# gphocs-dev/G-PhoCS

Measured on AMD Instinct MI355X. Metric: locus-likelihood evals/sec (+ MCMC iters/sec), 100k loci, 1/2/4/8 MI355X, higher is better.
Workload: dtype f64

## Files before the change

g-phocs_amd/__init__.py:

```python
import ctypes as C
import os
import subprocess

import numpy as np

from .synth import make_synthetic_pack, replicate_pack, write_pack

_HERE = os.path.dirname(os.path.abspath(__file__))
REPO = os.path.dirname(_HERE)
LIB_PATH = os.path.join(_HERE, "libgphocs_hip.so")
CSRC = os.path.join(_HERE, "csrc")

HIPCC_BASE = ["--offload-arch=gfx950", "-O3", "-std=c++17", "-ffp-contract=off", "-fPIC", "-shared",
              "-Wno-unused-result", "-pthread"]
HIPCC_TUNING = ["-mllvm", "-disable-machine-licm", "-mllvm", "-structurizecfg-skip-uniform-regions",
                "-mllvm", "-amdgpu-sched-strategy=max-ilp"]
HIPCC_TUNING_SPILLING = HIPCC_TUNING[:4]
HIPCC_FLAGS = HIPCC_BASE + HIPCC_TUNING
HIPCC_LIBS = ["-ldl", "-lrt"]
HIPCC_VALIDATED = "roc-7.2.0 26014"
PLAIN_LIB = "libgphocs_hip_plain.so"
CHECKED_LIB = "libgphocs_hip_chk.so"
CHECKED_LIB_BIG = "libgphocs_hip_chkb.so"

# ... 195 lines not shown
    "gph_control_sample_name", "gph_loci_read", "gph_loci_free", "gph_loci_arrays", "gph_run_control_file", "gph_run_control_file_ranked",
    "gph_read_trace", "gph_engine_locus_rate_update", "gph_engine_set_locus_rates", "gph_mcmc_set_locus_rate_finetune",
    "gph_mcmc_locus_rate_state", "gph_engine_set_comm", "gph_engine_host_stats", "gph_engine_set_timing",
    "gph_comm_unique_id", "gph_comm_create_rccl", "gph_comm_create_shm", "gph_comm_attach_shm", "gph_comm_shm_bytes",
    "gph_comm_destroy", "gph_comm_world", "gph_comm_rank", "gph_comm_on_stream", "gph_comm_kind",
    "gph_comm_allgather_stream", "gph_comm_allreduce_host", "gph_run_control_file_comm", "gph_device_count",
    "gph_engine_unit", "gph_build_id", "gph_build_compiler", "gph_runtime_version", "gph_engine_steplog_enable", "gph_engine_steplog_fetch", "gph_comm_local_group", "gph_comm_create_local",
    "gph_mcmc_get_chain", "gph_mcmc_set_chain", "gph_mcmc_update_gb", "gph_mcmc_update_locus_rate", "gph_mcmc_update_theta",
    "gph_mcmc_update_mig_rates", "gph_mcmc_update_tau", "gph_mcmc_update_sample_age", "gph_mcmc_mixing",
    "gph_mcmc_synchronize_events", "gph_mcmc_check_all", "gph_mcmc_initialize_genealogies",
    "gph_engine_locus_summary_enable", "gph_engine_locus_summary_sample", "gph_engine_locus_summary_columns",
    "gph_engine_locus_summary_fetch", "gph_engine_locus_summary_column_name", "gph_loci_name", "gph_run_control_file_ex",
    "gph_engine_coal_stats_enable", "gph_engine_coal_stats_sample", "gph_engine_coal_stats_shape", "gph_engine_coal_stats_fetch",
    "gph_engine_coal_stats_column_name", "gph_run_control_file_ex2", "gph_coal_stats_write", "gph_coal_stats_discard",
    "gph_engine_coal_stats_set_chunk", "gph_coal_stats_combined",
]


_LIBS = {}


def load_library(path=None, dims=None):
    if path is None and dims is not None:
        path = lib_path(variant_for(*dims))
    path = path or LIB_PATH
    if path in _LIBS:
        return _LIBS[path]
    lib = _load_library(path)
    _LIBS[path] = lib
    return lib
# ... 84 lines not shown
    lib.gph_engine_locus_summary_column_name.argtypes = [C.c_void_p, C.c_int32]
    lib.gph_engine_locus_summary_column_name.restype = C.c_char_p
    lib.gph_loci_name.argtypes = [C.c_void_p, C.c_int64]
    lib.gph_loci_name.restype = C.c_char_p
    lib.gph_run_control_file_ex.argtypes = [C.c_char_p, C.c_char_p, C.c_int32, C.c_int32, C.c_void_p, C.c_char_p]
    lib.gph_engine_coal_stats_enable.argtypes = [C.c_void_p, C.c_int32]
    lib.gph_engine_coal_stats_sample.argtypes = [C.c_void_p, C.c_int32]
    lib.gph_engine_coal_stats_shape.argtypes = [C.c_void_p] + [C.POINTER(C.c_int32)] * 4
    lib.gph_engine_coal_stats_fetch.argtypes = [C.c_void_p, C.POINTER(C.c_double), C.c_int32, C.POINTER(C.c_int32)]
    lib.gph_engine_coal_stats_column_name.argtypes = [C.c_void_p, C.c_int32]
    lib.gph_engine_coal_stats_column_name.restype = C.c_char_p
    lib.gph_run_control_file_ex2.argtypes = [C.c_char_p, C.c_char_p, C.c_int32, C.c_int32, C.c_void_p, C.c_char_p, C.c_char_p, C.c_int32]
    lib.gph_coal_stats_write.argtypes = [C.c_char_p, C.c_int32]
    lib.gph_coal_stats_discard.argtypes = [C.c_char_p, C.c_int32]
    lib.gph_engine_coal_stats_set_chunk.argtypes = [C.c_void_p, C.c_int32]
    lib.gph_coal_stats_combined.argtypes = [C.c_char_p, C.c_int32, C.POINTER(C.c_double), C.c_int64, C.POINTER(C.c_int64), C.POINTER(C.c_int32)]
    return lib


def encode_phases(counts):
    a = np.asarray(counts, dtype=np.int64)
    big = a >= 0x8000
    if big.any():
        ex = np.round(np.log2(np.where(big, a, 1))).astype(np.int64)
        assert np.all((1 << ex[big]) == a[big]), "a phase count of 2^15 or more must be a power of two"
        a = np.where(big, 0x8000 | ex, a)
    return a.astype(np.uint16)


def decode_phases(words):
# ... 332 lines not shown
    def last_kernel_ms(self, which):
        ms = C.c_double()
        self._chk(self.lib.gph_engine_last_kernel_ms(self.engine, which, C.byref(ms)), "kernel_ms")
        return ms.value

    def class_stats(self, which, reset=False):
        o = (C.c_double * 5)()
        self._chk(self.lib.gph_engine_class_stats(self.engine, which, o, int(reset)), "class_stats")
        return dict(launches=o[0], ms=o[1], evals=o[2], bytes=o[3], nodes=o[4])

    def host_stats(self):
        a, b, c, r = C.c_int64(), C.c_int64(), C.c_int64(), C.c_int32()
        self._chk(self.lib.gph_engine_host_stats(self.engine, C.byref(a), C.byref(b), C.byref(c), C.byref(r)), "host_stats")
        return dict(syncs=a.value, collectives=b.value, launches=c.value, resident=bool(r.value))

    def set_timing(self, mask):
        self._chk(self.lib.gph_engine_set_timing(self.engine, mask), "set_timing")

    def unit(self, op, arg=0):
        stride = max(13, 3 * (self.pack.n - 1), 1 + 5 * (2 * self.pack.n - 1))
        out = np.zeros((self.end - self.begin, stride))
        self._chk(self.lib.gph_engine_unit(self.engine, op, arg, out.ctypes.data_as(C.POINTER(C.c_double)), stride), "unit")
        return out

    def debug_oob(self):
        w, c = C.c_int32(), C.c_int32()
        self._chk(self.lib.gph_engine_debug_oob(self.engine, C.byref(w), C.byref(c)), "debug_oob")
        return w.value, c.value

    def enable_locus_summary(self, on=True):
# ... 66 lines not shown
```

g-phocs_amd/csrc/gph_engine.hip:

```cpp
#include <stdio.h>
#include <stdlib.h>
#include <stddef.h>
#include <string.h>
#include <vector>
#include <string>
#include <algorithm>
#if defined(GPH_HOSTEMU) && defined(GPH_EMU64)
#define GPH_EMU64_IMPL
#endif
#include "gph_kernels.h"
#include "gph_global.h"
#include "gph_summary.h"
#include "gph_coalstats.h"
#include "gph_comm.h"
#include "../../include/gphocs_hip.h"

#ifdef GPH_HOSTEMU
thread_local char *gph_sm = nullptr;
thread_local GphLds gph_lds;
GphLayout g_lay;
GphModel g_model;
GphGlobal *gph_G_emu = nullptr;
#ifdef GPH_BOUNDS
int gph_oob_word = 0;
// ... 326 lines not shown
  bool sync_pending = false;
  bool fin_owed = false;
  bool mix_owed = false;
  int32_t slog_sel = 0;
  bool mirror_current = true;
  bool no_fuse = false;
  gph_counters counters = {0, 0, 0.0, 0};
  double *d_ls = nullptr;
  int32_t ls_ncol = 0;
  int64_t ls_samples = 0;
  std::vector<std::string> ls_names;
  double *d_cs_part = nullptr, *d_cs_rows = nullptr;
  int32_t cs_cap = 0, cs_fill = 0, cs_rd = 0, cs_chunk = 0, cs_nchunks = 0, cs_bd = 0;
  int32_t cs_chunk_next = 0;
  std::string cs_name;
  double last_ms[16] = {0};
  double cls_launches[16] = {0}, cls_ms[16] = {0};
  double cls_evals0[16] = {0}, cls_bytes0[16] = {0}, cls_nodes0[16] = {0};
  int last_which = 0;
  uint32_t timing_mask = 0xffffffffu;
#ifndef GPH_HOSTEMU
  hipStream_t stream = nullptr;
  hipStream_t stream_wide = nullptr;
  hipEvent_t ev_fork = nullptr, ev_join = nullptr;
  bool side_stream = true;
  struct Tm { hipEvent_t a, b; int which; };
  std::vector<Tm> tm;
  size_t tm_used = 0;
#else
  std::vector<char> lds;
// ... 517 lines not shown
  e->popFather.assign(cfg->popFather, cfg->popFather + cfg->K);
  e->popSon0.assign(cfg->popSon0, cfg->popSon0 + cfg->K);
  e->popSon1.assign(cfg->popSon1, cfg->popSon1 + cfg->K);
  if (cfg->B > 0) { e->bandSrc.assign(cfg->bandSrc, cfg->bandSrc + cfg->B); e->bandTgt.assign(cfg->bandTgt, cfg->bandTgt + cfg->B); }
  e->cfg.samplesPerPop = e->samplesPerPop.data();
  e->cfg.popFather = e->popFather.data();
  e->cfg.popSon0 = e->popSon0.data();
  e->cfg.popSon1 = e->popSon1.data();
  e->cfg.bandSrc = e->bandSrc.data();
  e->cfg.bandTgt = e->bandTgt.data();
  memset(&e->dev, 0, sizeof e->dev);
  memset(&e->ka, 0, sizeof e->ka);
  fill_math_constants(e->ka);
  if (const char *fh = getenv("GPH_HOST_DECISIONS")) e->force_host = atoi(fh) != 0;
  if (const char *nf = getenv("GPH_NO_FUSE")) e->no_fuse = atoi(nf) != 0;
#ifndef GPH_HOSTEMU
  int ndev = 0;
  if (hipGetDeviceCount(&ndev) != hipSuccess || ndev <= cfg->device) {
    fprintf(stderr, "gphocs_hip: no usable HIP device %d (found %d) -- this library has no CPU path\n", cfg->device, ndev);
    delete e;
    return GPH_EHIP;
  }
  if (hipSetDevice(cfg->device) != hipSuccess || fill_math_tables(e->ka)) {
    fprintf(stderr, "gphocs_hip: cannot resolve the device math tables\n");
    delete e;
    return GPH_EHIP;
  }
  if (const char *ov = getenv("GPH_SIDE_STREAM")) e->side_stream = atoi(ov) != 0;
  const bool nb_ = getenv("GPH_NONBLOCKING_STREAM") && atoi(getenv("GPH_NONBLOCKING_STREAM")) != 0;
  if ((nb_ ? hipStreamCreateWithFlags(&e->stream, hipStreamNonBlocking) : hipStreamCreate(&e->stream)) != hipSuccess ||
// ... 15 lines not shown
  e->d_gather = e->d_red;
#endif
  memset(e->G_h, 0, sizeof(GphGlobal));
  e->G_h->error_locus = -1;
  build_model_static(e);
  *out = e;
  return 0;
}

void gph_engine_destroy(gph_engine *e)
{
  if (!e) return;
  dev_free(e->dev.pages); dev_free(e->dev.shadow); dev_free(e->dev.cond); dev_free((void *)e->dev.cond_off);
  dev_free((void *)e->dev.seq); dev_free((void *)e->dev.seq_off); dev_free((void *)e->dev.orig); dev_free((void *)e->dev.P); dev_free(e->dev.out); dev_free(e->dev.stats); dev_free(e->d_mutRate);
  dev_free(e->d_lrec); dev_free(e->d_lpre); dev_free(e->d_slot_of); dev_free(e->d_lr_result); dev_free(e->d_lr_gscr); dev_free(e->d_ref_page); dev_free(e->d_ref_seq);
  dev_free(e->d_part); dev_free(e->dev.err); dev_free(e->d_ls); dev_free(e->d_cs_part); dev_free(e->d_cs_rows);
  for (void *p : e->deferred_free) dev_free(p);
  e->deferred_free.clear();
  dev_free((void *)e->dev.slog_map); dev_free(e->dev.slog); dev_free(e->dev.slog_n);
  if (e->d_gather != e->d_red) dev_free(e->d_gather);
  dev_free(e->d_red);
#ifdef GPH_HOSTEMU
  free(e->h_red);
  free(e->G_h);
#else
  dev_free(e->G_d);
  dev_free(e->d_ticket);
  if (e->h_red) (void)hipHostFree(e->h_red);
  if (e->G_h) (void)hipHostFree(e->G_h);
  for (auto &t : e->tm) { (void)hipEventDestroy(t.a); (void)hipEventDestroy(t.b); }
  if (e->ev_fork) (void)hipEventDestroy(e->ev_fork);
// ... 270 lines not shown
  e->cs_fill = 0;
  LAUNCH(e, 3, k_init, e->seedz, (const double *)e->d_mutRate, e->init_predraws);
  int rc = reduce_local(e, 0, GPH_OUT_SLOTS);
  if (!rc) rc = reduce_stats(e);
  if (rc) return rc;
  e->G_h->nrec = 0;
  e->G_h->iteration = -1;
  if ((rc = run_stage_now(e, GS_INIT_DONE, 0))) return rc;
  { GphRed R; R.rows = e->h_red; R.world = 1;
    if (sumGen) *sumGen = R.sum(0, 0);
    if (sumData) *sumData = R.sum(0, 1); }
  e->initialized = true;
  return rc;
}

int gph_engine_genealogy_sweep(gph_engine *e, int32_t flags, double ftCoal, double ftMig, gph_sweep_result *out)
{
  if (!e || !e->initialized || !out) return GPH_ESTATE;
  SETDEV(e);
  PUSH_IF_DIRTY(e);
  const int with_sync = e->sync_pending ? 8 : 0;
  e->sync_pending = false;
  GphGlobal &G = *e->G_h;
  const double d0 = G.dataLogLikelihood, l0 = G.logLikelihood;
  const int64_t a0 = G.acc[0], a1 = G.acc[1], a2 = G.acc[2], a7 = G.acc[7];
  int with_mix = 0;
  if (e->mix_owed) {
    if (!e->mirror_current) { int rcm = finish_sync(e); if (rcm) return rcm; }
    e->mix_owed = false;
    if (e->G_h->mix_flag) with_mix = 16;
  }
  LAUNCH(e, 0, k_sweep, (int)flags | with_sync | with_mix, ftCoal, ftMig, e->G_h->mix_c, e->G_h->mix_lnc);
  int rc = reduce_local(e, 0, GPH_OUT_SLOTS);
  if (!rc) rc = reduce_stats(e);
  if (rc) return rc;
  if ((rc = run_stage_now(e, GS_SWEEP_DONE, with_sync))) return rc;
  GphRed R; R.rows = e->h_red; R.world = 1;
  out->accepted_internal = G.acc[0] - a0;
  out->accepted_mignode = G.acc[1] - a1;
  out->accepted_spr = G.acc[2] - a2;
  out->total_mig_nodes = G.acc[7] - a7;
  out->dData_internal = R.sum(0, 3);
  out->dLog_internal = R.sum(0, 4);
  out->dLog_mignode = R.sum(0, 5);
  out->dData_spr = R.sum(0, 6);
  out->dLog_spr = R.sum(0, 7);
// ... 232 lines not shown

int gph_engine_host_stats(gph_engine *e, int64_t *syncs, int64_t *collectives, int64_t *launches, int32_t *resident_mode)
{
  if (!e) return GPH_EARG;
  if (syncs) *syncs = e->n_syncs;
  if (collectives) *collectives = e->n_collectives;
  if (launches) *launches = e->n_launches;
  if (resident_mode) *resident_mode = resident(e) ? 1 : 0;
  return 0;
}
int gph_engine_set_timing(gph_engine *e, uint32_t class_mask)
{
  if (!e) return GPH_EARG;
  e->timing_mask = class_mask;
  return 0;
}

int gph_debug_math(const double *x, const double *y, int32_t n, double *out, int32_t device)
{
  if (!x || !y || !out || n <= 0) return GPH_EARG;
#ifdef GPH_HOSTEMU
  (void)device;
  for (int i = 0; i < n; i++) {
    out[i] = gph_exp(x[i]); out[n + i] = gph_log(x[i]); out[2 * n + i] = sqrt(fabs(x[i]));
    out[3 * n + i] = x[i] / y[i]; out[4 * n + i] = floor(x[i]);
  }
  return 0;
#else
  double *dx = nullptr, *dy = nullptr, *dout = nullptr;
  HIPCHK(hipSetDevice(device));
// ... 86 lines not shown
  *nrec = n;
#ifdef GPH_BBCOUNT
  n = e->dev.slog_cap;
#endif
  const int32_t m = std::min(std::min(n, e->dev.slog_cap), max_records);
  if (out && m > 0 && d2h(e, out, e->dev.slog + (size_t)idx * e->dev.slog_cap * 8, sizeof(double) * 8 * (size_t)m)) return GPH_EHIP;
  if (reset) { const int32_t z = 0; if (h2d(e, e->dev.slog_n + idx, &z, sizeof z)) return GPH_EHIP; }
  return 0;
#endif
}

int gph_engine_hbm_bytes(gph_engine *e, double *bytes)
{
  if (!e || !bytes) return GPH_EARG;
  *bytes = 2.0 * e->pages_bytes + (double)e->cond_bytes + (double)e->seq_bytes_total + 8.0 * GPH_OUT_SLOTS * e->L;
  return 0;
}

int gph_engine_set_locus_rates(gph_engine *e, const double *rates, int32_t draws, int32_t variable)
{
  if (!e || !e->loaded || e->initialized || !rates || draws < 0) return GPH_ESTATE;
  SETDEV(e);
  std::vector<double> r(e->L);
  for (int64_t j = 0; j < e->L; j++) r[j] = rates[e->h_orig[j]];
  if (!e->d_mutRate && dev_alloc((void **)&e->d_mutRate, sizeof(double) * e->L)) return GPH_EHIP;
  if (h2d(e, e->d_mutRate, r.data(), sizeof(double) * e->L)) return GPH_EHIP;
  e->init_predraws = draws;
  e->var_rates = variable != 0;
  return 0;
}
// ... 185 lines not shown
{
  if (e->fin_owed) { e->fin_owed = false; LAUNCH(e, 5, k_tau_finish, 0); }
  return 0;
}
static int part_sweep(gph_engine *e, int32_t iteration, double ftCoal, double ftMig)
{
  int rc;
  const int with_sync = e->sync_pending ? 8 : 0;
  e->sync_pending = false;
  int with_mix = 0;
  if (e->mix_owed) {
    if (!e->mirror_current) { int rcm = finish_sync(e); if (rcm) return rcm; }
    e->mix_owed = false;
    if (e->G_h->mix_flag) with_mix = 16;
  }
  LAUNCH(e, 0, k_sweep, 7 | with_sync | with_mix, ftCoal, ftMig, e->G_h->mix_c, e->G_h->mix_lnc);
  if ((rc = reduce_local(e, 0, GPH_OUT_SLOTS))) return rc;
  if ((rc = reduce_stats(e))) return rc;
  return run_stage(e, GS_SWEEP_DONE, with_sync, iteration);
}
static int part_lrate(gph_engine *e, int32_t iteration, const double *lr_alpha_finetune, int64_t *lr_accepted, double *lr_rateVar)
{
  int rc;
  GphGlobal &Gh = *e->G_h;
  gph_locus_rate_result R;
  R.accepted = 0; R.dataLogLikelihood = Gh.dataLogLikelihood; R.logLikelihood = Gh.logLikelihood; R.rateVar = *lr_rateVar;
  if ((rc = gph_engine_locus_rate_update(e, lr_alpha_finetune[1], lr_alpha_finetune[0], &R))) return rc;
  Gh.dataLogLikelihood = R.dataLogLikelihood; Gh.logLikelihood = R.logLikelihood; *lr_rateVar = R.rateVar;
  *lr_accepted += R.accepted;
  gg_rec(Gh, REC_LRATE, 0, (long long)R.accepted);
// ... 450 lines not shown
```

g-phocs_amd/csrc/gph_kernels.h:

```cpp
#pragma once
#include "gph_rt.h"

struct GphDev {
  char *pages;
  char *shadow;
  char *cond;
  const uint64_t *cond_off;
  const char *seq;
  const uint64_t *seq_off;
  const int32_t *P;
  const int32_t *orig;
  double *out;
  double *stats;
  int32_t L;
  int32_t Ltot;
  int64_t locus_begin;
  int32_t *err;
  const int32_t *slog_map;
  double *slog;
  int32_t *slog_n;
  int32_t slog_cap, pad_;
};

#include "gph_locus.h"
// ... 378 lines not shown
  OUT(g, 6, gf64(&GphLds::s_cntf, 5));
  OUT(g, 7, gf64(&GphLds::s_cntf, 6));
}

GPH_DEV void kb_sweep(const GphDev &D, int g, int flags, double ftCoal, double ftMig, double mix_c, double mix_lnc)
{
  STAMP_BEGIN(0);
  if (flags & 16) {
    stage_in_evaluated(D, g, 1);
    mix_commit_body(mix_c, mix_lnc);
  } else {
    stage_in(D, g, D.pages, 1);
  }
  GPH_SLOG_OPEN(D, g);
  GphRngB rng;
  rng_load(rng);
  OUT(g, 15, (flags & 8) ? (double)synchronize_events() : 1.0);
  OUT(g, 0, 0.0); OUT(g, 1, 0.0); OUT(g, 2, 0.0); OUT(g, 3, 0.0); OUT(g, 4, 0.0);
  OUT(g, 5, 0.0); OUT(g, 6, 0.0); OUT(g, 7, 0.0); OUT(g, 12, 0.0);
  { STAMP_BEGIN(5); if ((flags & 1) && ftCoal > 0.0) sweep_internal(D, g, ftCoal, rng); STAMP_END(5); }
  { STAMPC_BEGIN(4); if ((flags & 2) && ftMig > 0.0 && !gph_failed()) sweep_mignodes(D, g, ftMig, rng); STAMPC_END(4); }
  { STAMP_BEGIN(6); if ((flags & 4) && !gph_failed()) sweep_spr(D, g, rng); STAMP_END(6); }
  rng_store(rng);
  out_common(D, g);
  STAMP_END(0);
#if defined(GPH_STAMPS) && !defined(GPH_HOSTEMU)
  for (int k = 0; k < 8; k++) OUT(g, k, gph_lds.s_stamp[k]);
#endif
  stage_out(D, g, D.pages, 1);
}

// ... 823 lines not shown
```

g-phocs_amd/csrc/gph_locus.h:

```cpp
#pragma once
#include "gph_rt.h"

template <bool GPH_GM> struct GphCtxT {
#ifndef GPH_HOSTEMU
  GPH_DEV gph_cmodel &gmodel() const
  {
#if GPH_BIG_BANDS
    return *(gph_cmodel *)&(((gph_ckargs *)__builtin_amdgcn_kernarg_segment_ptr())->G->model);
#else
    if constexpr (GPH_GM) return *(gph_cmodel *)&(((gph_ckargs *)__builtin_amdgcn_kernarg_segment_ptr())->G->model);
    else return ((gph_ckargs *)__builtin_amdgcn_kernarg_segment_ptr())->model;
#endif
  }
#endif
  GphPad<IS_COUNT + CN_COUNT + SI_COUNT> r_pad;
#ifdef GPH_LOGSTEPS
  double *slog_ = nullptr;
  int32_t *slog_n_ = nullptr;
  int32_t slog_cap_ = 0;
  long long slog_gen_ = 0;
#define GPH_SLOG_OPEN(D, g) do { slog_ = nullptr; if ((D).slog_map && (D).slog_map[g] >= 0) { const int si_ = (D).slog_map[g]; \
      slog_ = (D).slog + (size_t)si_ * (D).slog_cap * 8; slog_n_ = (D).slog_n + si_; slog_cap_ = (D).slog_cap; } } while (0)
#define GPH_SLOG(kind, a, b, c, d, e, f) do { if (slog_ && GPH_LANE == 0) { const int k_ = (*slog_n_)++; if (k_ < slog_cap_) { double *r_ = slog_ + (size_t)k_ * 8; \
      r_[0] = (kind); r_[1] = (double)(a); r_[2] = (double)(b); r_[3] = (double)(c); r_[4] = (double)(d); r_[5] = (double)(e); r_[6] = (double)(f); r_[7] = 0.0; } } } while (0)
// ... 239 lines not shown
    const gph_cdbl *RC = GPH_RNGC;
    const double rx = RC[0], ry = RC[1], rz = RC[2], mx = RC[3], my = RC[4], mz = RC[5];
    double xd = (double)x, yd = (double)y, zd = (double)z, q;
    q = xd * rx; double qx = __builtin_fma(__builtin_fma(-q, mx, xd), rx, q);
    q = yd * ry; double qy = __builtin_fma(__builtin_fma(-q, my, yd), ry, q);
    q = zd * rz; double qz = __builtin_fma(__builtin_fma(-q, mz, zd), rz, q);
    r = qx + qy + qz;
  }
  return __builtin_amdgcn_fract(r);
#endif
  r = (r - (int)r);
  return r;
}
#ifdef GPH_HOSTEMU
typedef GphRng GphRngB;
#else
#ifndef GPH_RNG_BATCH
#define GPH_RNG_BATCH 16
#endif
struct GphRngB {
  int pos;
  double u;
};
GPH_DEV void rng_load(GphRngB &g)
{
  setCNT(CN_RX, ISC(IS_RX)); setCNT(CN_RY, ISC(IS_RY)); setCNT(CN_RZ, ISC(IS_RZ));
  g.pos = GPH_RNG_BATCH; g.u = 0.0;
}
GPH_DEV void rng_store(const GphRngB &g)
{
  uint32_t x = (uint32_t)CNT(CN_RX), y = (uint32_t)CNT(CN_RY), z = (uint32_t)CNT(CN_RZ);
  if (g.pos < GPH_RNG_BATCH) {
    x = (uint32_t)ISC(IS_RX); y = (uint32_t)ISC(IS_RY); z = (uint32_t)ISC(IS_RZ);
    for (int k = 0; k < g.pos; k++) {
      x = 171u * x - 30269u * (x / 177u);
      y = 172u * y - 30307u * (y / 176u);
      z = 170u * z - 30323u * (z / 178u);
    }
  }
  setISC(IS_RX, (int)x); setISC(IS_RY, (int)y); setISC(IS_RZ, (int)z);
}
#ifndef GPH_RNG_ROLLED
template <int K> GPH_DEV void rng_steps_(uint32_t &x, uint32_t &y, uint32_t &z, int &vx, int &vy, int &vz)
{
  if constexpr (K < GPH_RNG_BATCH) {
    x = 171u * x - 30269u * (x / 177u);
    y = 172u * y - 30307u * (y / 176u);
    z = 170u * z - 30323u * (z / 178u);
    asm("v_writelane_b32 %0, %3, %6\n\tv_writelane_b32 %1, %4, %6\n\tv_writelane_b32 %2, %5, %6"
        : "+v"(vx), "+v"(vy), "+v"(vz) : "s"(x), "s"(y), "s"(z), "i"(K));
    rng_steps_<K + 1>(x, y, z, vx, vy, vz);
  }
}
#endif
#ifndef GPH_RNG_VECTOR_REFILL
GPH_DEV void rng_refill(GphRngB &g)
{
  uint32_t x = (uint32_t)CNT(CN_RX), y = (uint32_t)CNT(CN_RY), z = (uint32_t)CNT(CN_RZ);
  int vx = 0, vy = 0, vz = 0;
  setISC(IS_RX, (int)x); setISC(IS_RY, (int)y); setISC(IS_RZ, (int)z);
#ifndef GPH_RNG_ROLLED
  rng_steps_<0>(x, y, z, vx, vy, vz);
#else
#pragma unroll 4
  for (int k = 0; k < GPH_RNG_BATCH; k++) {
    x = 171u * x - 30269u * (x / 177u);
    y = 172u * y - 30307u * (y / 176u);
    z = 170u * z - 30323u * (z / 178u);
    asm("s_mov_b32 m0, %6\n\ts_nop 0\n\tv_writelane_b32 %0, %3, m0\n\tv_writelane_b32 %1, %4, m0\n\tv_writelane_b32 %2, %5, m0"
        : "+v"(vx), "+v"(vy), "+v"(vz) : "s"(x), "s"(y), "s"(z), "s"(k) : "m0");
  }
#endif
  setCNT(CN_RX, (int)x); setCNT(CN_RY, (int)y); setCNT(CN_RZ, (int)z);
#if defined(__HIP_DEVICE_COMPILE__)
  {
    const gph_cdbl *RC = GPH_RNGC;
    const double rx = RC[0], ry = RC[1], rz = RC[2], mx = RC[3], my = RC[4], mz = RC[5];
    double xd = (double)(uint32_t)vx, yd = (double)(uint32_t)vy, zd = (double)(uint32_t)vz, q;
    q = xd * rx; double qx = __builtin_fma(__builtin_fma(-q, mx, xd), rx, q);
    q = yd * ry; double qy = __builtin_fma(__builtin_fma(-q, my, yd), ry, q);
    q = zd * rz; double qz = __builtin_fma(__builtin_fma(-q, mz, zd), rz, q);
    g.u = __builtin_amdgcn_fract(qx + qy + qz);
  }
#endif
  g.pos = 0;
}
#else
#define GPH_RNGV_STEP \
  "v_mul_hi_u32 %[q], %[st], %[mg]\n\t" \
// ... 2141 lines not shown
```

g-phocs_amd/csrc/gph_types.h:

```cpp
#pragma once
#include <stdint.h>

#ifndef GPH_CAP_LEAVES
#define GPH_CAP_LEAVES 24
#endif
#ifndef GPH_CAP_K
#define GPH_CAP_K 16
#endif
#ifndef GPH_CAP_B
#define GPH_CAP_B 8
#endif
#if GPH_CAP_K > 32
#define GPH_MAXK 40
typedef uint64_t gph_popmask;
#else
#define GPH_MAXK 32
typedef uint32_t gph_popmask;
#endif
#if GPH_CAP_B > 16
#define GPH_MAXB 100
#define GPH_BIG_BANDS 1
#else
#define GPH_MAXB 16
#define GPH_BIG_BANDS 0
// ... 47 lines not shown
  int32_t lds_sum;
  int32_t cnt16;
  int32_t dyn_bytes;
  int32_t huge_P;
};
struct GphGlobal;
struct GphKargs {
#if !GPH_BIG_BANDS
  GphModel model;
#endif
  GphLayout lay;
  double mathc[32];
  const double *log_t;
  const uint64_t *exp_t;
  GphGlobal *G;
};

#define GPH_PHASES(w) ((int)(w) < 0x8000 ? (int)(w) : (1 << ((int)(w) & 31)))
#define GPH_PHASES_ENCODE_MIN 0x8000
#define GPH_Q_LEAF 0
#define GPH_Q_NH(n) (((n) + 1) >> 1)
#define GPH_Q_PHASES(P, n) (((P) * GPH_Q_NH(n) + 1) & ~1)
#define GPH_Q_COUNT(P, n) ((GPH_Q_PHASES(P, n) + 2 * (P) + 3) & ~3)
#define GPH_Q_BYTES(P, n, c16) ((GPH_Q_COUNT(P, n) + ((c16) ? 2 : 4) * (P) + 15) & ~15)
#define GPH_Q_TERMS(P, n, c16) GPH_Q_BYTES(P, n, c16)
enum { DI_ORIG = 0, DI_UPD, DI_DLIN, DI_NEV, DI_NPOPS, DI_NBANDS, DI_SRCPOP, DI_TGTPOP, DI_COUNT };
enum { SI_FEV_OLD = 0, SI_FEV_NEW, SI_FPOP_NEW, SI_TARGET, SI_NOLD, SI_NNEW, SI_COUNT };
enum { SA_OLD = 0, SA_NEWIN, SA_NEWOUT, SA_NEWBAND };
enum { CN_EVALS = 0, CN_NODES, CN_ERROR, CN_P, CN_NOTENOUGH, CN_RX, CN_RY, CN_RZ, CN_EMPTY, CN_NODES0, CN_QPH, CN_QCNT, CN_QTERMS, CN_SUMLDS, CN_HUGE, CN_SEQLO, CN_SEQHI, CN_COUNT };

enum { FS_DATALNL = 0, FS_SV_DATALNL, FS_GENLNL, FS_GENDELTA, FS_MUTRATE, FS_COUNT };
enum { IS_ROOT = 0, IS_SV_ROOT, IS_DIRTY0, IS_CBIT0 = IS_DIRTY0 + GPH_NSW, IS_SAVED0 = IS_CBIT0 + GPH_NSW,
       IS_FREE = IS_SAVED0 + GPH_NSW, IS_NUM_MIGS, IS_RB_NUM, IS_CONFLICT_LOG, IS_RX, IS_RY, IS_RZ, IS_COUNT };
static_assert(IS_COUNT <= IS_COUNT_, "page scalars");
enum { MG_BRANCH = 0, MG_BAND, MG_SPOP, MG_TPOP, MG_SEV, MG_TEV, MG_COUNT };

#define GPH_OUT_SLOTS 16
enum { OUT_ACCEPT = 0, OUT_DDATA, OUT_DLOG, OUT_EVALS, OUT_EVALNODES, OUT_EVALBYTES,
       OUT_NTJ0, OUT_NTJ1, OUT_CONFLICT, OUT_ERROR, OUT_GENLNL, OUT_DATALNL, OUT_NMIGS };

#define GPH_CAP_N (2 * GPH_CAP_LEAVES - 1)
#define GPH_CAP_E (2 * GPH_CAP_LEAVES + 4 * GPH_MAX_MIGS + 3 * GPH_CAP_B + GPH_CAP_K + 10)
#define GPH_CAP_RB (GPH_MAX_MIGS + 2 * GPH_CAP_B)

// ... 122 lines not shown
```

include/gphocs_hip.h:

```cpp
#ifndef GPHOCS_HIP_H
#define GPHOCS_HIP_H
#include <stddef.h>
#include <stdint.h>
#ifdef __cplusplus
extern "C" {
#endif

#define GPH_OK 0
#define GPH_EARG (-1)
#define GPH_EHIP (-2)
#define GPH_EKERNEL (-3)
#define GPH_ESTATE (-4)
#define GPH_EFULL (-5)

typedef struct gph_engine gph_engine;
typedef struct gph_mcmc gph_mcmc;

typedef struct {
  int32_t n;
  int32_t Kc, K, B;
  int32_t rootPop;
  const int32_t *samplesPerPop;
  const int32_t *popFather, *popSon0, *popSon1;
  const int32_t *bandSrc, *bandTgt;
// ... 102 lines not shown
int gph_engine_steplog_fetch(gph_engine *e, int32_t idx, double *out, int32_t max_records, int32_t *nrec, int32_t reset);
const char *gph_build_compiler(void);
const char *gph_runtime_version(void);
int gph_engine_locus_summary_enable(gph_engine *e, int32_t on);
int gph_engine_locus_summary_sample(gph_engine *e);
int gph_engine_locus_summary_columns(gph_engine *e, int32_t *ncol, int64_t *samples);
int gph_engine_locus_summary_fetch(gph_engine *e, double *out, int64_t ld, int32_t reset);
const char *gph_engine_locus_summary_column_name(gph_engine *e, int32_t col);
int gph_engine_coal_stats_enable(gph_engine *e, int32_t capacity);
int gph_engine_coal_stats_sample(gph_engine *e, int32_t iteration);
int gph_engine_coal_stats_shape(gph_engine *e, int32_t *row_doubles, int32_t *filled, int32_t *n, int32_t *K);
int gph_engine_coal_stats_fetch(gph_engine *e, double *out, int32_t max_rows, int32_t *rows);
const char *gph_engine_coal_stats_column_name(gph_engine *e, int32_t col);
int gph_engine_coal_stats_set_chunk(gph_engine *e, int32_t slots);

typedef struct {
  const double *thetaAlpha, *thetaBeta, *thetaStart;
  const double *ageAlpha, *ageBeta, *ageStart;
  const double *sampleAge;
  const int32_t *updateSampleAge;
  const double *mrAlpha, *mrBeta;
  double ftCoalTime, ftMigTime, ftTheta, ftMigRate, ftMixing;
  const double *ftTaus;
  int32_t seed, startMig, doMixing, samplesPerLog;
  int32_t numParameters;
  const double *printFactors;
  int32_t mutRateMode;
  double varRatesAlpha, ftLocusRate;
} gph_mcmc_config;

// ... 83 lines not shown
```

Measured before the change: 433.8 million.

## Pregenerate per-locus RNG draws in a device pool consumed by sweep kernel

Adds a per-locus ring buffer of precomputed Wichmann-Hill RNG states, topped up before each genealogy sweep by a separate coalesced kernel. The sweep kernel then loads 16 states per batch in parallel across lanes instead of running the serial scalar recurrence with writelane. If the pool runs dry or its state does not match, it falls back to in-kernel generation. The goal is to take the serial RNG dependency chain off the latency-bound sweep. The cost is an extra launch per sweep, more device memory, and pool-consistency bookkeeping that could break RNG-stream equivalence if it is wrong.

```diff
diff --git a/g-phocs_amd/__init__.py b/g-phocs_amd/__init__.py
--- a/g-phocs_amd/__init__.py
+++ b/g-phocs_amd/__init__.py
@@ -233,6 +233,7 @@
     "gph_engine_coal_stats_enable", "gph_engine_coal_stats_sample", "gph_engine_coal_stats_shape", "gph_engine_coal_stats_fetch",
     "gph_engine_coal_stats_column_name", "gph_run_control_file_ex2", "gph_coal_stats_write", "gph_coal_stats_discard",
     "gph_engine_coal_stats_set_chunk", "gph_coal_stats_combined",
+    "gph_engine_rng_pool_set_capacity", "gph_engine_rng_pool_stats", "gph_debug_rng_pool_words", "gph_debug_rng_pool",
 ]
 
 
@@ -347,6 +348,11 @@
     lib.gph_coal_stats_write.argtypes = [C.c_char_p, C.c_int32]
     lib.gph_coal_stats_discard.argtypes = [C.c_char_p, C.c_int32]
     lib.gph_engine_coal_stats_set_chunk.argtypes = [C.c_void_p, C.c_int32]
+    lib.gph_engine_rng_pool_set_capacity.argtypes = [C.c_void_p, C.c_int32]
+    lib.gph_engine_rng_pool_stats.argtypes = [C.c_void_p, C.POINTER(C.c_int64)]
+    lib.gph_debug_rng_pool_words.restype = C.c_int64
+    lib.gph_debug_rng_pool_words.argtypes = [C.c_int32, C.c_int32]
+    lib.gph_debug_rng_pool.argtypes = [C.c_void_p, C.c_int32, C.c_int32, C.c_void_p, C.c_int32, C.c_void_p, C.c_void_p, C.c_int32]
     lib.gph_coal_stats_combined.argtypes = [C.c_char_p, C.c_int32, C.POINTER(C.c_double), C.c_int64, C.POINTER(C.c_int64), C.POINTER(C.c_int32)]
     return lib
 
@@ -709,6 +715,14 @@
         self._chk(self.lib.gph_engine_host_stats(self.engine, C.byref(a), C.byref(b), C.byref(c), C.byref(r)), "host_stats")
         return dict(syncs=a.value, collectives=b.value, launches=c.value, resident=bool(r.value))
 
+    def set_rng_pool(self, entries):
+        self._chk(self.lib.gph_engine_rng_pool_set_capacity(self.engine, int(entries)), "rng_pool_set_capacity")
+
+    def rng_pool_stats(self):
+        o = (C.c_int64 * 4)()
+        self._chk(self.lib.gph_engine_rng_pool_stats(self.engine, o), "rng_pool_stats")
+        return dict(capacity=o[0], mismatch=o[1], exhausted=o[2], regenerated=o[3])
+
     def set_timing(self, mask):
         self._chk(self.lib.gph_engine_set_timing(self.engine, mask), "set_timing")
 
diff --git a/g-phocs_amd/csrc/gph_engine.hip b/g-phocs_amd/csrc/gph_engine.hip
--- a/g-phocs_amd/csrc/gph_engine.hip
+++ b/g-phocs_amd/csrc/gph_engine.hip
@@ -364,6 +364,8 @@
   int32_t cs_cap = 0, cs_fill = 0, cs_rd = 0, cs_chunk = 0, cs_nchunks = 0, cs_bd = 0;
   int32_t cs_chunk_next = 0;
   std::string cs_name;
+  uint32_t *d_rng_pool = nullptr;
+  int32_t rng_cap = 0, rng_cap_next = GPH_RNG_POOL_DEFAULT;
   double last_ms[16] = {0};
   double cls_launches[16] = {0}, cls_ms[16] = {0};
   double cls_evals0[16] = {0}, cls_bytes0[16] = {0}, cls_nodes0[16] = {0};
@@ -911,6 +913,7 @@
   fill_math_constants(e->ka);
   if (const char *fh = getenv("GPH_HOST_DECISIONS")) e->force_host = atoi(fh) != 0;
   if (const char *nf = getenv("GPH_NO_FUSE")) e->no_fuse = atoi(nf) != 0;
+  if (const char *rp = getenv("GPH_RNG_POOL")) (void)gph_engine_rng_pool_set_capacity(e, atoi(rp));
 #ifndef GPH_HOSTEMU
   int ndev = 0;
   if (hipGetDeviceCount(&ndev) != hipSuccess || ndev <= cfg->device) {
@@ -956,7 +959,7 @@
   dev_free(e->dev.pages); dev_free(e->dev.shadow); dev_free(e->dev.cond); dev_free((void *)e->dev.cond_off);
   dev_free((void *)e->dev.seq); dev_free((void *)e->dev.seq_off); dev_free((void *)e->dev.orig); dev_free((void *)e->dev.P); dev_free(e->dev.out); dev_free(e->dev.stats); dev_free(e->d_mutRate);
   dev_free(e->d_lrec); dev_free(e->d_lpre); dev_free(e->d_slot_of); dev_free(e->d_lr_result); dev_free(e->d_lr_gscr); dev_free(e->d_ref_page); dev_free(e->d_ref_seq);
-  dev_free(e->d_part); dev_free(e->dev.err); dev_free(e->d_ls); dev_free(e->d_cs_part); dev_free(e->d_cs_rows);
+  dev_free(e->d_part); dev_free(e->dev.err); dev_free(e->d_ls); dev_free(e->d_cs_part); dev_free(e->d_cs_rows); dev_free(e->d_rng_pool);
   for (void *p : e->deferred_free) dev_free(p);
   e->deferred_free.clear();
   dev_free((void *)e->dev.slog_map); dev_free(e->dev.slog); dev_free(e->dev.slog_n);
@@ -1257,6 +1260,59 @@
   return rc;
 }
 
+int gph_engine_rng_pool_set_capacity(gph_engine *e, int32_t entries)
+{
+  if (!e || entries < 0) return GPH_EARG;
+  if (entries > GPH_RNG_POOL_MAX) entries = GPH_RNG_POOL_MAX;
+  e->rng_cap_next = (entries + GPH_RNG_BATCH - 1) / GPH_RNG_BATCH * GPH_RNG_BATCH;
+  return 0;
+}
+int gph_engine_rng_pool_stats(gph_engine *e, int64_t *out)
+{
+  if (!e || !out) return GPH_EARG;
+  out[0] = e->rng_cap; out[1] = out[2] = out[3] = 0;
+  if (!e->d_rng_pool) return 0;
+  SETDEV(e);
+  uint32_t st[RPS_COUNT];
+  if (d2h(e, st, e->d_rng_pool + (size_t)e->L * gph_rp_stride(e->rng_cap), sizeof st)) return GPH_EHIP;
+  out[1] = st[RPS_MISMATCH]; out[2] = st[RPS_EXHAUSTED]; out[3] = st[RPS_REGEN];
+  return 0;
+}
+static int rng_pool_topup(gph_engine *e)
+{
+  if (e->rng_cap != e->rng_cap_next) {
+    if (e->d_rng_pool) { if (stream_sync(e)) return GPH_EHIP; dev_free(e->d_rng_pool); e->d_rng_pool = nullptr; }
+    e->rng_cap = 0;
+    if (e->rng_cap_next > 0) {
+      const size_t words = gph_rp_words(e->L, e->rng_cap_next);
+      if (dev_alloc((void **)&e->d_rng_pool, 4 * words)) return GPH_EHIP;
+#ifdef GPH_HOSTEMU
+      memset(e->d_rng_pool, 0xff, 4 * (words - RPS_COUNT));
+      memset(e->d_rng_pool + words - RPS_COUNT, 0, 4 * RPS_COUNT);
+#else
+      HIPCHK(hipMemsetAsync(e->d_rng_pool, 0xff, 4 * (words - RPS_COUNT), e->stream));
+      HIPCHK(hipMemsetAsync(e->d_rng_pool + words - RPS_COUNT, 0, 4 * RPS_COUNT, e->stream));
+#endif
+      e->rng_cap = e->rng_cap_next;
+    }
+  }
+  e->ka.rng_pool = e->d_rng_pool; e->ka.rng_cap = e->rng_cap; e->ka.rng_slots = (int32_t)e->L;
+  if (!e->d_rng_pool) return 0;
+  const int L = (int)e->L, C = e->rng_cap;
+#ifdef GPH_HOSTEMU
+  uint32_t *stats = e->d_rng_pool + (size_t)L * gph_rp_stride(C);
+  for (int j = 0; j < L; j++) {
+    const int32_t *is = (const int32_t *)(e->dev.pages + (size_t)j * e->lay.page_bytes + e->lay.o_iscal);
+    stats[RPS_REGEN] += (uint32_t)gph_rp_topup_slot(e->d_rng_pool + (size_t)j * gph_rp_stride(C), C, (uint32_t)is[IS_RX], (uint32_t)is[IS_RY], (uint32_t)is[IS_RZ]);
+  }
+#else
+  hipLaunchKernelGGL(k_rng_pool, dim3((unsigned)((L + 63) / 64)), dim3(64), 0, e->stream, e->lay, (const char *)e->dev.pages, e->d_rng_pool, L, C);
+  HIPCHK(hipGetLastError());
+#endif
+  e->n_launches++;
+  return 0;
+}
+
 int gph_engine_genealogy_sweep(gph_engine *e, int32_t flags, double ftCoal, double ftMig, gph_sweep_result *out)
 {
   if (!e || !e->initialized || !out) return GPH_ESTATE;
@@ -1273,6 +1329,7 @@
     e->mix_owed = false;
     if (e->G_h->mix_flag) with_mix = 16;
   }
+  { int rcp = rng_pool_topup(e); if (rcp) return rcp; }
   LAUNCH(e, 0, k_sweep, (int)flags | with_sync | with_mix, ftCoal, ftMig, e->G_h->mix_c, e->G_h->mix_lnc);
   int rc = reduce_local(e, 0, GPH_OUT_SLOTS);
   if (!rc) rc = reduce_stats(e);
@@ -1535,6 +1592,22 @@
   if (!e) return GPH_EARG;
   e->timing_mask = class_mask;
   return 0;
+}
+
+int64_t gph_debug_rng_pool_words(int32_t nslots, int32_t entries) { return nslots < 0 || entries < 0 ? -1 : (int64_t)gph_rp_words(nslots, entries); }
+int32_t gph_debug_rng_pool(uint32_t *pool, int32_t nslots, int32_t entries, uint32_t *states, int32_t op, const int32_t *ndraws, uint32_t *out, int32_t cap)
+{
+  if (!pool || !states || nslots < 0 || entries <= 0 || entries % GPH_RNG_BATCH) return -1;
+  int32_t n = 0;
+  for (int j = 0; j < nslots; j++) {
+    uint32_t *slot = pool + (size_t)j * gph_rp_stride(entries), *st = states + 3 * (size_t)j;
+    if (op == 0) n += gph_rp_topup_slot(slot, entries, st[0], st[1], st[2]);
+    else {
+      if (!ndraws || !out || ndraws[j] < 0 || ndraws[j] > cap) return -1;
+      n += gph_rp_consume_slot(slot, entries, st[0], st[1], st[2], ndraws[j], out + 3 * (size_t)j * cap) != 0;
+    }
+  }
+  return n;
 }
 
 int gph_debug_math(const double *x, const double *y, int32_t n, double *out, int32_t device)
@@ -1651,6 +1724,7 @@
 {
   if (!e || !bytes) return GPH_EARG;
   *bytes = 2.0 * e->pages_bytes + (double)e->cond_bytes + (double)e->seq_bytes_total + 8.0 * GPH_OUT_SLOTS * e->L;
+  if (e->rng_cap_next > 0) *bytes += 4.0 * (double)gph_rp_words(e->L, e->rng_cap_next);
   return 0;
 }
 
@@ -1866,6 +1940,7 @@
     e->mix_owed = false;
     if (e->G_h->mix_flag) with_mix = 16;
   }
+  if ((rc = rng_pool_topup(e))) return rc;
   LAUNCH(e, 0, k_sweep, 7 | with_sync | with_mix, ftCoal, ftMig, e->G_h->mix_c, e->G_h->mix_lnc);
   if ((rc = reduce_local(e, 0, GPH_OUT_SLOTS))) return rc;
   if ((rc = reduce_stats(e))) return rc;
diff --git a/g-phocs_amd/csrc/gph_kernels.h b/g-phocs_amd/csrc/gph_kernels.h
--- a/g-phocs_amd/csrc/gph_kernels.h
+++ b/g-phocs_amd/csrc/gph_kernels.h
@@ -1,5 +1,6 @@
 #pragma once
 #include "gph_rt.h"
+#include "gph_rngpool.h"
 
 struct GphDev {
   char *pages;
@@ -416,7 +417,7 @@
   }
   GPH_SLOG_OPEN(D, g);
   GphRngB rng;
-  rng_load(rng);
+  rng_load_sweep(rng, g);
   OUT(g, 15, (flags & 8) ? (double)synchronize_events() : 1.0);
   OUT(g, 0, 0.0); OUT(g, 1, 0.0); OUT(g, 2, 0.0); OUT(g, 3, 0.0); OUT(g, 4, 0.0);
   OUT(g, 5, 0.0); OUT(g, 6, 0.0); OUT(g, 7, 0.0); OUT(g, 12, 0.0);
diff --git a/g-phocs_amd/csrc/gph_locus.h b/g-phocs_amd/csrc/gph_locus.h
--- a/g-phocs_amd/csrc/gph_locus.h
+++ b/g-phocs_amd/csrc/gph_locus.h
@@ -277,6 +277,7 @@
 }
 #ifdef GPH_HOSTEMU
 typedef GphRng GphRngB;
+GPH_DEV void rng_load_sweep(GphRngB &g, int slot) { (void)slot; rng_load(g); }
 #else
 #ifndef GPH_RNG_BATCH
 #define GPH_RNG_BATCH 16
@@ -285,13 +286,51 @@
   int pos;
   double u;
 };
-GPH_DEV void rng_load(GphRngB &g)
+#define GPH_RP_BASE(slot, C) ((const GPH_GLB uint32_t *)GPH_KA->rng_pool + (size_t)(uint32_t)(slot) * gph_rp_stride(C))
+GPH_DEV void rng_load_sweep(GphRngB &g, int slot)
 {
   setCNT(CN_RX, ISC(IS_RX)); setCNT(CN_RY, ISC(IS_RY)); setCNT(CN_RZ, ISC(IS_RZ));
   g.pos = GPH_RNG_BATCH; g.u = 0.0;
+  setCNT(CN_PSLOT, slot); setCNT(CN_PAVAIL, -1); setCNT(CN_PN, 0);
+#if defined(__HIP_DEVICE_COMPILE__) && !defined(GPH_RNG_VECTOR_REFILL)
+  const int C = GPH_KA->rng_cap;
+  if (C > 0) {
+    const int w = (int)GPH_RP_BASE(slot, C)[GPH_LANE & (GPH_RP_HDR - 1)];
+    const bool ok = __builtin_amdgcn_readlane(w, RP_FRESH) == 0 && __builtin_amdgcn_readlane(w, RP_SX) == ISC(IS_RX) &&
+                    __builtin_amdgcn_readlane(w, RP_SY) == ISC(IS_RY) && __builtin_amdgcn_readlane(w, RP_SZ) == ISC(IS_RZ) &&
+                    (uint32_t)__builtin_amdgcn_readlane(w, RP_CUR) < (uint32_t)C && (uint32_t)__builtin_amdgcn_readlane(w, RP_FILL) <= (uint32_t)C;
+    if (ok) {
+      const int fill = __builtin_amdgcn_readlane(w, RP_FILL);
+      setCNT(CN_PCUR, __builtin_amdgcn_readlane(w, RP_CUR)); setCNT(CN_PAVAIL, fill); setCNT(CN_PN, fill);
+    } else {
+      setCNT(CN_PN, 1 + RPS_MISMATCH);
+    }
+  }
+#endif
 }
 GPH_DEV void rng_store(const GphRngB &g)
 {
+#if defined(__HIP_DEVICE_COMPILE__)
+  const int avail = CNT(CN_PAVAIL);
+  if (avail >= 0) {
+    if (CNT(CN_PN) != avail) {
+      const int C = GPH_KA->rng_cap, back = GPH_RNG_BATCH - g.pos;
+      int idx = CNT(CN_PCUR) - back - 1;
+      if (idx < 0) idx += C;
+      const GPH_GLB uint32_t *h = GPH_RP_BASE(CNT(CN_PSLOT), C), *t = h + GPH_RP_HDR + 3 * idx;
+      const int x = RFL(t[0]), y = RFL(t[1]), z = RFL(t[2]);
+      setISC(IS_RX, x); setISC(IS_RY, y); setISC(IS_RZ, z);
+      if (GPH_LANE == 0) {
+        GPH_GLB uint32_t *hw = (GPH_GLB uint32_t *)h;
+        hw[RP_CUR] = (uint32_t)(idx + 1 == C ? 0 : idx + 1); hw[RP_FILL] = (uint32_t)(avail + back);
+        hw[RP_SX] = (uint32_t)x; hw[RP_SY] = (uint32_t)y; hw[RP_SZ] = (uint32_t)z;
+      }
+    }
+    return;
+  }
+  if (CNT(CN_PN) != 0 && GPH_LANE == 0)
+    atomicAdd((uint32_t *)GPH_KA->rng_pool + (size_t)GPH_KA->rng_slots * gph_rp_stride(GPH_KA->rng_cap) + (CNT(CN_PN) - 1), 1u);
+#endif
   uint32_t x = (uint32_t)CNT(CN_RX), y = (uint32_t)CNT(CN_RY), z = (uint32_t)CNT(CN_RZ);
   if (g.pos < GPH_RNG_BATCH) {
     x = (uint32_t)ISC(IS_RX); y = (uint32_t)ISC(IS_RY); z = (uint32_t)ISC(IS_RZ);
@@ -303,29 +342,25 @@
   }
   setISC(IS_RX, (int)x); setISC(IS_RY, (int)y); setISC(IS_RZ, (int)z);
 }
-#ifndef GPH_RNG_ROLLED
-template <int K> GPH_DEV void rng_steps_(uint32_t &x, uint32_t &y, uint32_t &z, int &vx, int &vy, int &vz)
-{
-  if constexpr (K < GPH_RNG_BATCH) {
-    x = 171u * x - 30269u * (x / 177u);
-    y = 172u * y - 30307u * (y / 176u);
-    z = 170u * z - 30323u * (z / 178u);
-    asm("v_writelane_b32 %0, %3, %6\n\tv_writelane_b32 %1, %4, %6\n\tv_writelane_b32 %2, %5, %6"
-        : "+v"(vx), "+v"(vy), "+v"(vz) : "s"(x), "s"(y), "s"(z), "i"(K));
-    rng_steps_<K + 1>(x, y, z, vx, vy, vz);
-  }
-}
-#endif
 #ifndef GPH_RNG_VECTOR_REFILL
-GPH_DEV void rng_refill(GphRngB &g)
-{
+GPH_DEV void rng_refill_inkernel(int &vx, int &vy, int &vz)
+{
+#if defined(__HIP_DEVICE_COMPILE__)
+  const int avail = CNT(CN_PAVAIL);
+  if (avail >= 0) {
+    if (CNT(CN_PN) != avail) {
+      const int C = GPH_KA->rng_cap;
+      int idx = CNT(CN_PCUR) - 1;
+      if (idx < 0) idx += C;
+      const GPH_GLB uint32_t *t = GPH_RP_BASE(CNT(CN_PSLOT), C) + GPH_RP_HDR + 3 * idx;
+      setCNT(CN_RX, RFL(t[0])); setCNT(CN_RY, RFL(t[1])); setCNT(CN_RZ, RFL(t[2]));
+    }
+    setCNT(CN_PAVAIL, -1); setCNT(CN_PN, 1 + RPS_EXHAUSTED);
+  }
+#endif
   uint32_t x = (uint32_t)CNT(CN_RX), y = (uint32_t)CNT(CN_RY), z = (uint32_t)CNT(CN_RZ);
-  int vx = 0, vy = 0, vz = 0;
   setISC(IS_RX, (int)x); setISC(IS_RY, (int)y); setISC(IS_RZ, (int)z);
-#ifndef GPH_RNG_ROLLED
-  rng_steps_<0>(x, y, z, vx, vy, vz);
-#else
-#pragma unroll 4
+#pragma unroll 1
   for (int k = 0; k < GPH_RNG_BATCH; k++) {
     x = 171u * x - 30269u * (x / 177u);
     y = 172u * y - 30307u * (y / 176u);
@@ -333,9 +368,24 @@
     asm("s_mov_b32 m0, %6\n\ts_nop 0\n\tv_writelane_b32 %0, %3, m0\n\tv_writelane_b32 %1, %4, m0\n\tv_writelane_b32 %2, %5, m0"
         : "+v"(vx), "+v"(vy), "+v"(vz) : "s"(x), "s"(y), "s"(z), "s"(k) : "m0");
   }
-#endif
   setCNT(CN_RX, (int)x); setCNT(CN_RY, (int)y); setCNT(CN_RZ, (int)z);
+}
+GPH_DEV void rng_refill(GphRngB &g)
+{
+  int vx = 0, vy = 0, vz = 0;
 #if defined(__HIP_DEVICE_COMPILE__)
+  const int avail = CNT(CN_PAVAIL);
+  if (__builtin_expect(avail >= GPH_RNG_BATCH, 1)) {
+    const int C = GPH_KA->rng_cap, cur = CNT(CN_PCUR);
+    int idx = cur + (GPH_LANE & (GPH_RNG_BATCH - 1));
+    if (idx >= C) idx -= C;
+    const GPH_GLB uint32_t *t = GPH_RP_BASE(CNT(CN_PSLOT), C) + GPH_RP_HDR + 3 * idx;
+    vx = (int)t[0]; vy = (int)t[1]; vz = (int)t[2];
+    const int nc = cur + GPH_RNG_BATCH;
+    setCNT(CN_PCUR, nc >= C ? nc - C : nc); setCNT(CN_PAVAIL, avail - GPH_RNG_BATCH);
+  } else {
+    rng_refill_inkernel(vx, vy, vz);
+  }
   {
     const gph_cdbl *RC = GPH_RNGC;
     const double rx = RC[0], ry = RC[1], rz = RC[2], mx = RC[3], my = RC[4], mz = RC[5];
diff --git a/g-phocs_amd/csrc/gph_rngpool.h b/g-phocs_amd/csrc/gph_rngpool.h
--- /dev/null
+++ b/g-phocs_amd/csrc/gph_rngpool.h
@@ -0,0 +1,140 @@
+#pragma once
+#include "gph_types.h"
+
+#ifndef GPH_RNG_BATCH
+#define GPH_RNG_BATCH 16
+#endif
+#define GPH_RP_HDR 16
+enum { RP_CUR = 0, RP_FILL, RP_SX, RP_SY, RP_SZ, RP_TX, RP_TY, RP_TZ, RP_FRESH };
+enum { RPS_MISMATCH = 0, RPS_EXHAUSTED, RPS_REGEN, RPS_COUNT = 4 };
+#ifndef GPH_RNG_POOL_DEFAULT
+#define GPH_RNG_POOL_DEFAULT 512
+#endif
+#define GPH_RNG_POOL_MAX 4096
+
+#if defined(GPH_HOSTEMU) || !defined(__HIPCC__)
+#define GPH_RP_HD static inline
+#else
+#define GPH_RP_HD __host__ __device__ inline
+#endif
+
+GPH_RP_HD size_t gph_rp_stride(int C) { return (size_t)GPH_RP_HDR + 3 * (size_t)C; }
+GPH_RP_HD size_t gph_rp_words(int64_t L, int C) { return (size_t)L * gph_rp_stride(C) + RPS_COUNT; }
+GPH_RP_HD void gph_rp_step(uint32_t &x, uint32_t &y, uint32_t &z)
+{
+  x = 171u * x - 30269u * (x / 177u);
+  y = 172u * y - 30307u * (y / 176u);
+  z = 170u * z - 30323u * (z / 178u);
+}
+GPH_RP_HD int gph_rp_topup_begin(uint32_t *h, int C, uint32_t px, uint32_t py, uint32_t pz, int &at, uint32_t &x, uint32_t &y, uint32_t &z, int &regen)
+{
+  regen = h[RP_FRESH] != 0 || h[RP_SX] != px || h[RP_SY] != py || h[RP_SZ] != pz || h[RP_CUR] >= (uint32_t)C || h[RP_FILL] > (uint32_t)C ||
+          (h[RP_CUR] + h[RP_FILL]) % GPH_RNG_BATCH != 0;
+  if (regen) {
+    h[RP_CUR] = 0; h[RP_FILL] = 0; h[RP_FRESH] = 0;
+    h[RP_SX] = px; h[RP_SY] = py; h[RP_SZ] = pz;
+    h[RP_TX] = px; h[RP_TY] = py; h[RP_TZ] = pz;
+  }
+  const int cur = (int)h[RP_CUR], fill = (int)h[RP_FILL];
+  at = (cur + fill) % C;
+  x = h[RP_TX]; y = h[RP_TY]; z = h[RP_TZ];
+  return (C - fill) / GPH_RNG_BATCH;
+}
+GPH_RP_HD void gph_rp_topup_end(uint32_t *h, int nb, uint32_t x, uint32_t y, uint32_t z)
+{
+  h[RP_FILL] += (uint32_t)(nb * GPH_RNG_BATCH);
+  h[RP_TX] = x; h[RP_TY] = y; h[RP_TZ] = z;
+}
+static inline int gph_rp_topup_slot(uint32_t *slot, int C, uint32_t px, uint32_t py, uint32_t pz)
+{
+  int at, regen;
+  uint32_t x, y, z;
+  const int nb = gph_rp_topup_begin(slot, C, px, py, pz, at, x, y, z, regen);
+  uint32_t *ring = slot + GPH_RP_HDR;
+  for (int b = 0; b < nb; b++) {
+    for (int k = 0; k < GPH_RNG_BATCH; k++) {
+      gph_rp_step(x, y, z);
+      uint32_t *t = ring + 3 * (size_t)(at + k);
+      t[0] = x; t[1] = y; t[2] = z;
+    }
+    at += GPH_RNG_BATCH;
+    if (at >= C) at = 0;
+  }
+  gph_rp_topup_end(slot, nb, x, y, z);
+  return regen;
+}
+static inline int gph_rp_consume_slot(uint32_t *slot, int C, uint32_t &px, uint32_t &py, uint32_t &pz, int ndraws, uint32_t *out)
+{
+  uint32_t *ring = slot + GPH_RP_HDR;
+  int rc = 0, k = 0;
+  if (C <= 0 || slot[RP_FRESH] != 0 || slot[RP_SX] != px || slot[RP_SY] != py || slot[RP_SZ] != pz) rc = 1;
+  else {
+    int cur = (int)slot[RP_CUR], avail = (int)slot[RP_FILL];
+    while (k < ndraws && avail >= GPH_RNG_BATCH) {
+      const int take = ndraws - k < GPH_RNG_BATCH ? ndraws - k : GPH_RNG_BATCH;
+      for (int i = 0; i < take; i++) {
+        const uint32_t *t = ring + 3 * (size_t)((cur + i) % C);
+        out[3 * (k + i)] = px = t[0]; out[3 * (k + i) + 1] = py = t[1]; out[3 * (k + i) + 2] = pz = t[2];
+      }
+      k += take;
+      if (take == GPH_RNG_BATCH) { cur = (cur + GPH_RNG_BATCH) % C; avail -= GPH_RNG_BATCH; }
+      else { cur = (cur + take) % C; avail -= take; }
+    }
+    if (k == ndraws) {
+      slot[RP_CUR] = (uint32_t)cur; slot[RP_FILL] = (uint32_t)avail;
+      slot[RP_SX] = px; slot[RP_SY] = py; slot[RP_SZ] = pz;
+      return 0;
+    }
+    rc = 2;
+  }
+  for (; k < ndraws; k++) {
+    gph_rp_step(px, py, pz);
+    out[3 * k] = px; out[3 * k + 1] = py; out[3 * k + 2] = pz;
+  }
+  return rc;
+}
+
+#if !defined(GPH_HOSTEMU) && defined(__HIPCC__)
+#define GPH_RP_TILE_ROW (3 * GPH_RNG_BATCH + 1)
+__global__ void __launch_bounds__(64) k_rng_pool(GphLayout y, const char *pages, uint32_t *pool, int L, int C)
+{
+  __shared__ uint32_t tile[64 * GPH_RP_TILE_ROW];
+  __shared__ int32_t tpos[64];
+  const int lane = threadIdx.x, j = blockIdx.x * 64 + lane;
+  const size_t stride = gph_rp_stride(C);
+  uint32_t *stats = pool + (size_t)L * stride;
+  uint32_t *h = pool + (size_t)(j < L ? j : L - 1) * stride;
+  int nb = 0, at = 0, regen = 0;
+  uint32_t x = 0, yy = 0, z = 0;
+  if (j < L) {
+    const int32_t *is = (const int32_t *)(pages + (size_t)j * y.page_bytes + y.o_iscal);
+    nb = gph_rp_topup_begin(h, C, (uint32_t)is[IS_RX], (uint32_t)is[IS_RY], (uint32_t)is[IS_RZ], at, x, yy, z, regen);
+    if (regen) atomicAdd(&stats[RPS_REGEN], 1u);
+  }
+  const int nb0 = nb;
+  const size_t wave_base = (size_t)blockIdx.x * 64 * stride + GPH_RP_HDR;
+  for (int done = 0; __any(done < nb); done++) {
+    const bool on = done < nb;
+    if (on) {
+#pragma unroll
+      for (int k = 0; k < GPH_RNG_BATCH; k++) {
+        gph_rp_step(x, yy, z);
+        tile[lane * GPH_RP_TILE_ROW + 3 * k] = x;
+        tile[lane * GPH_RP_TILE_ROW + 3 * k + 1] = yy;
+        tile[lane * GPH_RP_TILE_ROW + 3 * k + 2] = z;
+      }
+    }
+    tpos[lane] = on ? at : -1;
+    if (on) { at += GPH_RNG_BATCH; if (at >= C) at = 0; }
+    __syncthreads();
+#pragma unroll 4
+    for (int t = 0; t < 3 * GPH_RNG_BATCH; t++) {
+      const int i = t * 64 + lane, r = i / (3 * GPH_RNG_BATCH), w = i - r * (3 * GPH_RNG_BATCH);
+      const int p = tpos[r];
+      if (p >= 0) pool[wave_base + (size_t)r * stride + 3 * (size_t)p + w] = tile[r * GPH_RP_TILE_ROW + w];
+    }
+    __syncthreads();
+  }
+  if (j < L) gph_rp_topup_end(h, nb0, x, yy, z);
+}
+#endif
diff --git a/g-phocs_amd/csrc/gph_types.h b/g-phocs_amd/csrc/gph_types.h
--- a/g-phocs_amd/csrc/gph_types.h
+++ b/g-phocs_amd/csrc/gph_types.h
@@ -85,6 +85,8 @@
   const double *log_t;
   const uint64_t *exp_t;
   GphGlobal *G;
+  uint32_t *rng_pool;
+  int32_t rng_cap, rng_slots;
 };
 
 #define GPH_PHASES(w) ((int)(w) < 0x8000 ? (int)(w) : (1 << ((int)(w) & 31)))
@@ -98,7 +100,7 @@
 enum { DI_ORIG = 0, DI_UPD, DI_DLIN, DI_NEV, DI_NPOPS, DI_NBANDS, DI_SRCPOP, DI_TGTPOP, DI_COUNT };
 enum { SI_FEV_OLD = 0, SI_FEV_NEW, SI_FPOP_NEW, SI_TARGET, SI_NOLD, SI_NNEW, SI_COUNT };
 enum { SA_OLD = 0, SA_NEWIN, SA_NEWOUT, SA_NEWBAND };
-enum { CN_EVALS = 0, CN_NODES, CN_ERROR, CN_P, CN_NOTENOUGH, CN_RX, CN_RY, CN_RZ, CN_EMPTY, CN_NODES0, CN_QPH, CN_QCNT, CN_QTERMS, CN_SUMLDS, CN_HUGE, CN_SEQLO, CN_SEQHI, CN_COUNT };
+enum { CN_EVALS = 0, CN_NODES, CN_ERROR, CN_P, CN_NOTENOUGH, CN_RX, CN_RY, CN_RZ, CN_EMPTY, CN_NODES0, CN_QPH, CN_QCNT, CN_QTERMS, CN_SUMLDS, CN_HUGE, CN_SEQLO, CN_SEQHI, CN_PSLOT, CN_PCUR, CN_PAVAIL, CN_PN, CN_COUNT };
 
 enum { FS_DATALNL = 0, FS_SV_DATALNL, FS_GENLNL, FS_GENDELTA, FS_MUTRATE, FS_COUNT };
 enum { IS_ROOT = 0, IS_SV_ROOT, IS_DIRTY0, IS_CBIT0 = IS_DIRTY0 + GPH_NSW, IS_SAVED0 = IS_CBIT0 + GPH_NSW,
diff --git a/include/gphocs_hip.h b/include/gphocs_hip.h
--- a/include/gphocs_hip.h
+++ b/include/gphocs_hip.h
@@ -140,6 +140,12 @@
 const char *gph_engine_coal_stats_column_name(gph_engine *e, int32_t col);
 int gph_engine_coal_stats_set_chunk(gph_engine *e, int32_t slots);
 
+int gph_engine_rng_pool_set_capacity(gph_engine *e, int32_t entries);
+int gph_engine_rng_pool_stats(gph_engine *e, int64_t out[4]);
+int64_t gph_debug_rng_pool_words(int32_t nslots, int32_t entries);
+int32_t gph_debug_rng_pool(uint32_t *pool, int32_t nslots, int32_t entries, uint32_t *states, int32_t op, const int32_t *ndraws,
+                           uint32_t *out, int32_t cap);
+
 typedef struct {
   const double *thetaAlpha, *thetaBeta, *thetaStart;
   const double *ageAlpha, *ageBeta, *ageStart;
```

Result: no change. 435.5 million, median of 6 (+0.4%).
